# cvxopt/cvxopt

Hardware: NVIDIA H100
Metric: kkt_factor_solve_gflops_fp64 (higher is better)
Workload: dtype f64

## Files before the change

### cvxopt_b200/csrc/chol.cu

```cuda
#include "common.cuh"
#include <cstdlib>

namespace cvxb {

namespace {

constexpr int PB = 8;
constexpr int SP = 12;
constexpr int LDM = NB + 4;
constexpr int POTF2_SMEM = (NB * LDM + NB * SP + 4 * 80) * 8;
constexpr int kGroup = 4;

template <int PAT>
__device__ __forceinline__ void sym_update(double (&acc)[4][8][2], const double *Ma, const double *Mb) {
#pragma unroll 2
    for (int kk = 0; kk < NB / 4; ++kk) {
        double a[4], bfr[8];
#pragma unroll
        for (int cf = 0; cf < 4; ++cf) a[cf] = -Ma[cf * 8 + kk * 4 * LDM];
#pragma unroll
        for (int rf = 0; rf < 8; ++rf) bfr[rf] = Mb[rf * 8 + kk * 4 * LDM];
#pragma unroll
        for (int mf = 0; mf < 2; ++mf)
#pragma unroll
            for (int rf = 0; rf < 8; ++rf) {
                if (PAT == 1 && rf < 2 * mf) continue;
                if (PAT == 2 && rf < 4 + 2 * mf) continue;
                dmma16x8x4(acc[2 * mf][rf][0], acc[2 * mf][rf][1], acc[2 * mf + 1][rf][0], acc[2 * mf + 1][rf][1],
                           a[2 * mf], a[2 * mf + 1], bfr[rf]);
            }
    }
}

__global__ void __launch_bounds__(256, 1)
potf2_inv_kernel(double *A, long long lda, int jb, double *inv, double *invT, int *info, int joff,
                 long long sA, long long sInv, const double *Tprev, long long ldt,
                 const double *invprev, unsigned long long *trace) {
    extern __shared__ __align__(16) double sm[];
    if (trace && threadIdx.x == 0) {
        unsigned long long t; asm volatile("mov.u64 %0, %%globaltimer;" : "=l"(t)); trace[0] = t;
    }
#define CVXB_STAMP(SLOT)                                                                    \
    if (trace && threadIdx.x == 0) {                                                        \
        unsigned long long t_; asm volatile("mov.u64 %0, %%globaltimer;" : "=l"(t_));       \
        trace[8 * 2048 + (SLOT)] = t_;                                                      \
    }
    A += (long long)blockIdx.x * sA; inv += (long long)blockIdx.x * sInv;
    invT += (long long)blockIdx.x * sInv; info += blockIdx.x;
    double *M = sm;
    double *P = M + NB * LDM;
    double *Dw = P + NB * SP;
    const int tid = threadIdx.x, lane = tid & 31, warp = tid >> 5;
    const int role = (0x72640531 >> (warp * 4)) & 7;
    const int wr = role & 1, wc = role >> 1;
    const int g4 = lane >> 2, t4 = lane & 3;

    double acc[4][8][2];
    if (Tprev != nullptr) {
#pragma unroll
        for (int cf = 0; cf < 4; ++cf)
#pragma unroll
            for (int rf = 0; rf < 8; ++rf) acc[cf][rf][0] = acc[cf][rf][1] = 0.0;
        const int kkmax = (wc + 1) * 8;
        {
            const bool v16 = ((ldt & 1) == 0) && ((reinterpret_cast<uintptr_t>(Tprev) & 15) == 0);
            if (v16) {
                for (int q = tid; q < NB * NB / 2; q += 256) {
                    const int c = q >> 6, r = (q & 63) * 2;
                    const int nb = (r + 1 < jb) ? 16 : (r < jb ? 8 : 0);
                    cp_async16(M + r + c * LDM, nb ? Tprev + r + (long long)c * ldt : Tprev, nb);
                }
            } else {
                for (int q = tid; q < NB * NB; q += 256) {
                    const int c = q >> 7, r = q & 127;
                    cp_async8(M + r + c * LDM, (r < jb) ? Tprev + r + (long long)c * ldt : Tprev, (r < jb) ? 8 : 0);
                }
            }
            cp_async_commit();
        }
        const double *ip = invprev + (wc * 32 + g4) + t4 * NB;
        double a0[4];
#pragma unroll
        for (int cf = 0; cf < 4; ++cf) a0[cf] = ip[cf * 8];
        cp_async_wait<0>();
        __syncthreads();
        const double *tq = M + (wr * 64 + g4) + t4 * LDM;
#pragma unroll 2
        for (int kk = 0; kk < kkmax; ++kk) {
            double a[4], bfr[8];
#pragma unroll
            for (int cf = 0; cf < 4; ++cf) a[cf] = a0[cf];
            if (kk + 1 < kkmax) {
#pragma unroll
                for (int cf = 0; cf < 4; ++cf) a0[cf] = ip[cf * 8 + (kk + 1) * 4 * NB];
            }
#pragma unroll
            for (int rf = 0; rf < 8; ++rf) bfr[rf] = tq[rf * 8 + kk * 4 * LDM];
#pragma unroll
            for (int mf = 0; mf < 2; ++mf)
#pragma unroll
                for (int rf = 0; rf < 8; ++rf)
                    dmma16x8x4(acc[2 * mf][rf][0], acc[2 * mf][rf][1], acc[2 * mf + 1][rf][0],
                               acc[2 * mf + 1][rf][1], a[2 * mf], a[2 * mf + 1], bfr[rf]);
        }
        __syncthreads();
#pragma unroll
        for (int cf = 0; cf < 4; ++cf)
#pragma unroll
            for (int rf = 0; rf < 8; ++rf)
#pragma unroll
                for (int e = 0; e < 2; ++e)
                    M[(wr * 64 + rf * 8 + t4 * 2 + e) + (wc * 32 + cf * 8 + g4) * LDM] = acc[cf][rf][e];
    }
    CVXB_STAMP(0)
#pragma unroll
    for (int cf = 0; cf < 4; ++cf)
#pragma unroll
        for (int rf = 0; rf < 8; ++rf)
#pragma unroll
            for (int e = 0; e < 2; ++e) {
                const int r = wr * 64 + rf * 8 + t4 * 2 + e, c = wc * 32 + cf * 8 + g4;
                double v = (r == c) ? 1.0 : 0.0;
                if (r < jb && c < jb && r >= c) v = A[r + (long long)c * lda];
                acc[cf][rf][e] = v;
            }
    __syncthreads();
    CVXB_STAMP(4)
    if (Tprev != nullptr) {
        const int d = wc - 2 * wr;
        const double *Ma = M + (wc * 32 + g4) + t4 * LDM;
        const double *Mb = M + (wr * 64 + g4) + t4 * LDM;
        if (d < 0) sym_update<0>(acc, Ma, Mb);
        else if (d == 0) sym_update<1>(acc, Ma, Mb);
        else if (d == 1) sym_update<2>(acc, Ma, Mb);
        __syncthreads();
    }
    CVXB_STAMP(1)
#pragma unroll 1
    for (int t = 0; t < NB / PB; ++t) {
      {
        const int c0 = t * PB;
        if (wc == (t >> 2)) {
#define CVXB_PUBLISH(CF)                                                          \
    _Pragma("unroll") for (int rf = 0; rf < 8; ++rf)                              \
        _Pragma("unroll") for (int e = 0; e < 2; ++e)                             \
            P[(wr * 64 + rf * 8 + t4 * 2 + e) * SP + g4] = acc[CF][rf][e];
            switch (t & 3) {
                case 0: CVXB_PUBLISH(0) break;
                case 1: CVXB_PUBLISH(1) break;
                case 2: CVXB_PUBLISH(2) break;
                default: CVXB_PUBLISH(3) break;
            }
#undef CVXB_PUBLISH
        }
        __syncthreads();
        if (warp == 0 && lane == 0) {
            double a[PB][PB];
#pragma unroll
            for (int i = 0; i < PB; ++i)
#pragma unroll
                for (int k = 0; k <= i; ++k) a[i][k] = P[(c0 + i) * SP + k];
            bool bad = false;
#pragma unroll
            for (int j = 0; j < PB; ++j) {
                const double piv = a[j][j];
                if (!(piv > 0.0) && !bad) {
                    atomicCAS(info, 0, joff + c0 + j + 1);
                    bad = true;
                }
                const double rs = rsqrt(piv);
                a[j][j] = piv * rs;
                Dw[64 + j] = rs;
#pragma unroll
                for (int i = j + 1; i < PB; ++i) a[i][j] *= rs;
#pragma unroll
                for (int k = j + 1; k < PB; ++k)
#pragma unroll
                    for (int i = k; i < PB; ++i) a[i][k] -= a[i][j] * a[k][j];
            }
#pragma unroll
            for (int i = 0; i < PB; ++i)
#pragma unroll
                for (int k = 0; k < PB; ++k) Dw[i * 8 + k] = (k <= i) ? a[i][k] : 0.0;
        }
        if (warp < 4) asm volatile("bar.sync 1, 128;" ::: "memory");
        if (warp < 4) {
            const double *D = Dw;
            const int r = warp * 32 + lane;
            double x[PB];
            if (r >= c0 + PB) {
#pragma unroll
                for (int j = 0; j < PB; ++j) x[j] = P[r * SP + j];
#pragma unroll
                for (int j = 0; j < PB; ++j) {
                    double v = x[j];
#pragma unroll
                    for (int k = 0; k < j; ++k) v -= x[k] * D[j * 8 + k];
                    x[j] = v * D[64 + j];
                }
            } else if (r >= c0) {
#pragma unroll
                for (int j = 0; j < PB; ++j) x[j] = (j <= r - c0) ? D[(r - c0) * 8 + j] : 0.0;
            } else {
#pragma unroll
                for (int j = 0; j < PB; ++j) x[j] = 0.0;
            }
#pragma unroll
            for (int j = 0; j < PB; ++j) P[r * SP + j] = x[j];
        }
        __syncthreads();
        if (wr * 8 + 7 > t && wc * 4 + 3 > t) {
            double a[4][2], bfr[8][2];
#pragma unroll
            for (int kk = 0; kk < 2; ++kk) {
#pragma unroll
                for (int cf = 0; cf < 4; ++cf) a[cf][kk] = -P[(wc * 32 + cf * 8 + g4) * SP + kk * 4 + t4];
#pragma unroll
                for (int rf = 0; rf < 8; ++rf) bfr[rf][kk] = P[(wr * 64 + rf * 8 + g4) * SP + kk * 4 + t4];
            }
#pragma unroll
            for (int mf = 0; mf < 2; ++mf) {
                if (wc * 4 + 2 * mf + 1 <= t) continue;
#pragma unroll
                for (int rf = 0; rf < 8; ++rf) {
                    dmma16x8x4(acc[2 * mf][rf][0], acc[2 * mf][rf][1], acc[2 * mf + 1][rf][0], acc[2 * mf + 1][rf][1],
                               a[2 * mf][0], a[2 * mf + 1][0], bfr[rf][0]);
                    dmma16x8x4(acc[2 * mf][rf][0], acc[2 * mf][rf][1], acc[2 * mf + 1][rf][0], acc[2 * mf + 1][rf][1],
                               a[2 * mf][1], a[2 * mf + 1][1], bfr[rf][1]);
                }
            }
        }
        for (int e = tid; e < NB * PB; e += 256) {
            const int r = e & (NB - 1), j = e >> 7;
            const double v = P[r * SP + j];
            M[r + (c0 + j) * LDM] = v;
            if (r >= c0 + j && r < jb && c0 + j < jb) A[r + (long long)(c0 + j) * lda] = v;
        }
        __syncthreads();
      }
    }

    CVXB_STAMP(2)
    {
        const int blk = warp * 2 + (lane >> 4);
        const int j = lane & 15;
        const int o = blk * PB;
        double x[PB];
        if (j < PB) {
#pragma unroll
            for (int i = 0; i < PB; ++i) {
                double v = (i == j) ? 1.0 : 0.0;
#pragma unroll
                for (int k = 0; k < i; ++k)
                    if (k >= j) v -= M[(o + i) + (o + k) * LDM] * x[k];
                x[i] = (i >= j) ? v / M[(o + i) + (o + i) * LDM] : 0.0;
            }
        }
        __syncwarp();
        if (j < PB) {
#pragma unroll
            for (int i = 0; i < PB; ++i) M[(o + i) + (o + j) * LDM] = x[i];
        }
    }
    __syncthreads();
    for (int s = PB; s < NB; s <<= 1) {
        const int sb = s / PB;
        const int tp = sb * sb;
        const int ntiles = (NB / (2 * s)) * tp;
#pragma unroll 1
        for (int phase = 0; phase < 2; ++phase) {
            for (int base = warp * 4; base < ntiles; base += 32) {
                double c[4][2];
                int oo[4], ti[4], tj[4];
#pragma unroll
                for (int u = 0; u < 4; ++u) {
                    const int idx = min(base + u, ntiles - 1);
                    const int pr = idx / tp, loc = idx - pr * tp;
                    ti[u] = loc % sb; tj[u] = loc / sb; oo[u] = pr * 2 * s;
                    c[u][0] = c[u][1] = 0.0;
                }
                for (int kb = 0; kb < sb; ++kb) {
#pragma unroll
                    for (int u = 0; u < 4; ++u) {
                        const bool live = phase == 0 ? (kb >= tj[u]) : (kb <= ti[u]);
                        if (!live) continue;
                        const int o = oo[u];
#pragma unroll
                        for (int kk = 0; kk < 2; ++kk) {
                            const int k = kb * 8 + kk * 4 + t4;
                            double af, bf;
                            if (phase == 0) {
                                af = M[(o + s + ti[u] * 8 + g4) + (o + k) * LDM];
                                bf = M[(o + k) + (o + tj[u] * 8 + g4) * LDM];
                            } else {
                                af = M[(o + s + ti[u] * 8 + g4) + (o + s + k) * LDM];
                                bf = M[(o + k) + (o + s + tj[u] * 8 + g4) * LDM];
                            }
                            dmma(c[u][0], c[u][1], af, bf);
                        }
                    }
                }
#pragma unroll
                for (int u = 0; u < 4; ++u) {
                    if (base + u >= ntiles) continue;
                    const int o = oo[u];
                    if (phase == 0) {
                        M[(o + ti[u] * 8 + g4) + (o + s + tj[u] * 8 + t4 * 2) * LDM] = c[u][0];
                        M[(o + ti[u] * 8 + g4) + (o + s + tj[u] * 8 + t4 * 2 + 1) * LDM] = c[u][1];
                    } else {
                        M[(o + s + ti[u] * 8 + g4) + (o + tj[u] * 8 + t4 * 2) * LDM] = -c[u][0];
                        M[(o + s + ti[u] * 8 + g4) + (o + tj[u] * 8 + t4 * 2 + 1) * LDM] = -c[u][1];
                    }
                }
            }
            __syncthreads();
        }
    }
    CVXB_STAMP(3)
    for (int e = tid; e < NB * NB; e += 256) {
        int i = e & (NB - 1), k = e >> 7;
        inv[e] = (i >= k) ? M[i + k * LDM] : 0.0;
        invT[e] = (k >= i) ? M[k + i * LDM] : 0.0;
    }
    if (trace && threadIdx.x == 0) {
        unsigned long long t; asm volatile("mov.u64 %0, %%globaltimer;" : "=l"(t)); trace[1] = t;
    }
}

constexpr int TR_CH = 32;
constexpr int TR_R = 5;
constexpr int TRSV_SMEM = (TR_R * NB * TR_CH + 4 * NB + 32 * 129) * 8;

template <bool TRANS, bool VEC>
__global__ void __launch_bounds__(256, 1)
trsv_kernel(int n, const double *__restrict__ L, long long ldl, const double *__restrict__ inv,
            const double *__restrict__ invT, double *b, int *flags, int epoch, long long sL,
            long long sInv, long long sb) {
    extern __shared__ __align__(16) double sm[];
    {
        const long long pb = blockIdx.y;
        L += pb * sL; inv += pb * sInv; invT += pb * sInv; b += pb * sb;
        flags += pb * ((n + NB - 1) / NB);
    }
    double *ring = sm;
    double *xs = ring + TR_R * NB * TR_CH;
    double *part = xs + NB;
    double *tvec = part + 2 * NB;
    double *part2 = tvec + NB;
    const int nblk = (n + NB - 1) / NB;
    const int tid = threadIdx.x, lane = tid & 31, warp = tid >> 5;
    const int bi = TRANS ? (nblk - 1 - (int)blockIdx.x) : (int)blockIdx.x;
    const int i0 = bi * NB;
    const int ni = min(NB, n - i0);
    const int r = tid & (NB - 1), half = tid >> 7;

    double ireg[64];
    {
        const double *ip = (TRANS ? invT : inv) + (long long)bi * NB * NB + r + (long long)(half * 64) * NB;
#pragma unroll
        for (int k = 0; k < 64; ++k) ireg[k] = ip[k * NB];
    }

    const double bown = (tid < ni) ? b[i0 + tid] : 0.0;
    const int nb_dep = TRANS ? (nblk - 1 - bi) : bi;
    const int nchunks = nb_dep * (NB / TR_CH);
    auto issue = [&](int q) {
        const int jj = q / (NB / TR_CH), cc = q % (NB / TR_CH);
        const int j = TRANS ? (nblk - 1 - jj) : jj;
        double *dst = ring + (q % TR_R) * (NB * TR_CH);
        const double *src;
        int nrows, ncols;
        if (!TRANS) { src = L + i0 + (long long)(j * NB + cc * TR_CH) * ldl; nrows = ni; ncols = TR_CH; }
        else { src = L + (long long)j * NB + (long long)(i0 + cc * TR_CH) * ldl; nrows = min(NB, n - j * NB); ncols = min(TR_CH, ni - cc * TR_CH); }
        if (VEC) {
#pragma unroll
            for (int it = 0; it < 8; ++it) {
                const int e = tid + it * 256;
                const int c = e >> 6, rr = (e & 63) * 2;
                const int rem = nrows - rr;
                const int bytes = (c < ncols) ? (rem >= 2 ? 16 : (rem == 1 ? 8 : 0)) : 0;
                cp_async16(dst + c * NB + rr, bytes ? (src + rr + (long long)c * ldl) : L, bytes);
            }
        } else {
#pragma unroll
            for (int it = 0; it < 16; ++it) {
                const int e = tid + it * 256;
                const int c = e >> 7, rr = e & 127;
                const int bytes = (c < ncols && rr < nrows) ? 8 : 0;
                cp_async8(dst + c * NB + rr, bytes ? (src + rr + (long long)c * ldl) : L, bytes);
            }
        }
    };
#pragma unroll
    for (int q = 0; q < TR_R - 1; ++q) {
        if (q < nchunks) issue(q);
        cp_async_commit();
    }

    double acc = 0.0;
    double accc[16];
#pragma unroll
    for (int q = 0; q < 16; ++q) accc[q] = 0.0;

    for (int jj = 0; jj < nb_dep; ++jj) {
        const int j = TRANS ? (nblk - 1 - jj) : jj;
        if (tid == 0) while (ld_acquire(flags + j) != epoch) { }
        __syncthreads();
        if (tid < NB) xs[tid] = (j * NB + tid < n) ? __ldcg(b + j * NB + tid) : 0.0;
#pragma unroll
        for (int cc = 0; cc < NB / TR_CH; ++cc) {
            const int q = jj * (NB / TR_CH) + cc;
            cp_async_wait<TR_R - 2>();
            __syncthreads();
            {
                const int nq = q + TR_R - 1;
                if (nq < nchunks) issue(nq);
                cp_async_commit();
            }
            const double *ch = ring + (q % TR_R) * (NB * TR_CH);
            if (!TRANS) {
#pragma unroll
                for (int c = 0; c < 16; ++c)
                    acc += ch[(half * 16 + c) * NB + r] * xs[cc * TR_CH + half * 16 + c];
            } else {
#pragma unroll
                for (int qc = 0; qc < 4; ++qc) {
                    const double *col = ch + (warp * 4 + qc) * NB;
                    double a = 0.0;
#pragma unroll
                    for (int rr = 0; rr < 4; ++rr) a += col[lane + rr * 32] * xs[lane + rr * 32];
                    accc[cc * 4 + qc] += a;
                }
            }
        }
    }
    cp_async_wait<0>();
    __syncthreads();
    if (!TRANS) {
        part[half * NB + r] = acc;
        __syncthreads();
        if (tid < NB) tvec[tid] = (tid < ni) ? (bown - part[tid] - part[NB + tid]) : 0.0;
        __syncthreads();
    } else {
#pragma unroll
        for (int q = 0; q < 16; ++q) {
            const int c = (q >> 2) * TR_CH + warp * 4 + (q & 3);
            part2[lane * 129 + c] = accc[q];
        }
        __syncthreads();
        if (tid < NB) {
            double sacc = 0.0;
#pragma unroll 8
            for (int l = 0; l < 32; ++l) sacc += part2[l * 129 + tid];
            tvec[tid] = (tid < ni) ? (bown - sacc) : 0.0;
        }
        __syncthreads();
    }
    double a2 = 0.0;
#pragma unroll
    for (int k = 0; k < 64; ++k) a2 += ireg[k] * tvec[half * 64 + k];
    part[half * NB + r] = a2;
    __syncthreads();
    if (tid < ni) b[i0 + tid] = part[tid] + part[NB + tid];
    __threadfence();
    __syncthreads();
    if (tid == 0) st_release(flags + bi, epoch);
}

std::atomic<int> g_trsv_epoch{0};

__global__ void __launch_bounds__(256)
transpose_panel_kernel(const double *__restrict__ W, long long ldw, int rows, double *__restrict__ WT, long long ldt) {
    __shared__ double t[32][33];
    const int r0 = blockIdx.x * 32, k0 = blockIdx.y * 32, tx = threadIdx.x, ty = threadIdx.y;
#pragma unroll
    for (int i = ty; i < 32; i += 8)
        if (r0 + tx < rows) t[i][tx] = W[r0 + tx + (long long)(k0 + i) * ldw];
    __syncthreads();
#pragma unroll
    for (int i = ty; i < 32; i += 8)
        if (r0 + i < rows) WT[k0 + tx + (long long)(r0 + i) * ldt] = t[tx][i];
}

}

int chol_work_create(CholWork &w) {
    int least = 0, greatest = 0;
    CVXB_CUDA(cudaDeviceGetStreamPriorityRange(&least, &greatest));
    CVXB_CUDA(cudaStreamCreateWithPriority(&w.panel_stream, cudaStreamNonBlocking, greatest));
    CVXB_CUDA(cudaStreamCreateWithPriority(&w.trsm_stream, cudaStreamNonBlocking, greatest));
    CVXB_CUDA(cudaStreamCreateWithPriority(&w.update_stream, cudaStreamNonBlocking, least));
    CVXB_CUDA(cudaStreamCreateWithPriority(&w.near_stream, cudaStreamNonBlocking, greatest));
    CVXB_CUDA(cudaEventCreateWithFlags(&w.ev_end_t, cudaEventDisableTiming));
    CVXB_CUDA(cudaEventCreateWithFlags(&w.ev_end_n, cudaEventDisableTiming));
    CVXB_CUDA(cudaEventCreateWithFlags(&w.ev_start, cudaEventDisableTiming));
    CVXB_CUDA(cudaEventCreateWithFlags(&w.ev_end_p, cudaEventDisableTiming));
    CVXB_CUDA(cudaEventCreateWithFlags(&w.ev_end_u, cudaEventDisableTiming));
    CVXB_TRY(w.d_info.alloc(1));
    CVXB_CUDA(cudaMemset(w.d_info.p, 0, sizeof(int)));
    CVXB_TRY(w.d_flags.alloc(4096));
    CVXB_CUDA(cudaMemset(w.d_flags.p, 0, 4096 * sizeof(int)));
    CVXB_TRY(w.splitk_ws.alloc(dmma_gemm_splitk_ws_doubles()));
    CVXB_CUDA(cudaFuncSetAttribute(potf2_inv_kernel, cudaFuncAttributeMaxDynamicSharedMemorySize,
                                   POTF2_SMEM));
    CVXB_CUDA(cudaFuncSetAttribute(trsv_kernel<true, true>, cudaFuncAttributeMaxDynamicSharedMemorySize, TRSV_SMEM));
    CVXB_CUDA(cudaFuncSetAttribute(trsv_kernel<true, false>, cudaFuncAttributeMaxDynamicSharedMemorySize, TRSV_SMEM));
    CVXB_CUDA(cudaFuncSetAttribute(trsv_kernel<false, true>, cudaFuncAttributeMaxDynamicSharedMemorySize, TRSV_SMEM));
    CVXB_CUDA(cudaFuncSetAttribute(trsv_kernel<false, false>, cudaFuncAttributeMaxDynamicSharedMemorySize, TRSV_SMEM));
    return 0;
}

CholWork::~CholWork() {
    for (cudaStream_t s : {panel_stream, update_stream, trsm_stream, near_stream}) if (s) cudaStreamDestroy(s);
    for (auto &g : graphs) if (g.exec) cudaGraphExecDestroy(g.exec);
    for (cudaEvent_t e : {ev_end_t, ev_end_n, ev_start, ev_end_p, ev_end_u}) if (e) cudaEventDestroy(e);
    for (auto *v : {&ev_dg, &ev_tr, &ev_c0, &ev_na, &ev_nb, &ev_n})
        for (cudaEvent_t e : *v) cudaEventDestroy(e);
}

static int potrf_enqueue(int n, double *A, int lda, double *inv, CholWork &w, cudaStream_t st) {
    if (n <= 0) return 0;
    const int nblk = (n + NB - 1) / NB;
    if (w.panel_rows < n) {
        for (auto &g : w.graphs) if (g.exec) cudaGraphExecDestroy(g.exec);
        w.graphs.clear();
        for (DevBuf<double> &pb : w.panel) pb.reset();
        for (DevBuf<double> &gb : w.group) gb.reset();
        const int rows = (n + 1) & ~1;
        for (DevBuf<double> &pb : w.panel) CVXB_TRY(pb.alloc((size_t)rows * NB));
        for (DevBuf<double> &gb : w.group) CVXB_TRY(gb.alloc((size_t)rows * kGroup * NB));
        w.panel_rows = rows;
    }
    while ((int)w.ev_dg.size() < nblk) {
        cudaEvent_t e[6];
        for (int i = 0; i < 6; ++i) CVXB_CUDA(cudaEventCreateWithFlags(&e[i], cudaEventDisableTiming));
        w.ev_dg.push_back(e[0]); w.ev_tr.push_back(e[1]); w.ev_c0.push_back(e[2]);
        w.ev_na.push_back(e[3]); w.ev_nb.push_back(e[4]); w.ev_n.push_back(e[5]);
    }
    if (getenv("CVXB_TRACE") && !w.trace.p) CVXB_TRY(w.trace.alloc(8 * 4096));
    unsigned long long *trace = w.trace.p;
    if (trace) CVXB_CUDA(cudaMemsetAsync(trace, 0, 8 * 4096 * sizeof(unsigned long long), st));
    const int ldw = w.panel_rows;
    const int ldg = kGroup * NB;
    cudaStream_t D = w.panel_stream, T = w.trsm_stream, U = w.update_stream, N = w.near_stream;
    CVXB_CUDA(cudaMemsetAsync(w.d_info.p, 0, sizeof(int), st));
    CVXB_CUDA(cudaEventRecord(w.ev_start, st));
    for (cudaStream_t s : {D, T, U, N}) CVXB_CUDA(cudaStreamWaitEvent(s, w.ev_start, 0));
    auto update = [&](int lo, int hi, const double *X, int ldx, bool kmajor, int K, unsigned long long *tr,
                      cudaStream_t s) -> int {
        double *Acc = A + (long long)lo * NB * (1 + (long long)lda);
        GemmDesc u;
        u.M = n - lo * NB; u.N = (hi * NB < n ? hi * NB : n) - lo * NB; u.K = K;
        u.X = X; u.ldx = ldx; u.x_kmajor = kmajor;
        u.Y = X; u.ldy = ldx; u.y_kmajor = kmajor;
        u.D = Acc; u.ldd = lda; u.C = Acc; u.ldc = lda;
        u.alpha = -1.0; u.beta = 1.0; u.lower_only = true;
        u.trace = tr;
        return dmma_gemm(u, s);
    };
    auto wait_col = [&](cudaStream_t s, int c) -> int {
        const int p = c - 2, g0 = kGroup * (c / kGroup);
        if (p < 0) return 0;
        if (p >= g0) CVXB_CUDA(cudaStreamWaitEvent(s, w.ev_na[p], 0));
        if (g0 > 0) CVXB_CUDA(cudaStreamWaitEvent(s, w.ev_nb[p < g0 - 1 ? p : g0 - 1], 0));
        return 0;
    };
    for (int jb = 0; jb < nblk; ++jb) {
        const int j = jb * NB;
        const int wj = (n - j < NB) ? (n - j) : NB;
        const int m = n - j - wj;
        double *Ajj = A + j + (long long)j * lda;
        double *invj = inv + (long long)jb * NB * NB;
        double *invTj = inv + (long long)(nblk + jb) * NB * NB;
        double *Wp = w.panel[jb & 1].p;
        if (jb >= 2) CVXB_CUDA(cudaStreamWaitEvent(D, w.ev_c0[jb - 2], 0));
        CVXB_TRY(wait_col(D, jb));
        const double *Tprev = jb > 0 ? A + j + (long long)(j - NB) * lda : nullptr;
        const double *invprev = jb > 0 ? inv + (long long)(jb - 1) * NB * NB : nullptr;
        potf2_inv_kernel<<<1, 256, POTF2_SMEM, D>>>(Ajj, lda, wj, invj, invTj, w.d_info.p, j, 0, 0, Tprev,
                                                     lda, invprev, trace ? trace + 8 * jb : nullptr);
        count_launch();
        CVXB_LAUNCH_CHECK();
        CVXB_CUDA(cudaEventRecord(w.ev_dg[jb], D));
        auto copy_back_prev = [&]() -> int {
            if (jb == 0) return 0;
            const int jp = j - NB, mp = n - j;
            CVXB_CUDA(cudaMemcpy2DAsync(A + j + (long long)jp * lda, (size_t)lda * sizeof(double),
                                        w.panel[(jb - 1) & 1].p, (size_t)ldw * sizeof(double),
                                        (size_t)mp * sizeof(double), NB, cudaMemcpyDeviceToDevice, T));
            return 0;
        };
        if (m <= 0) {
            CVXB_CUDA(cudaStreamWaitEvent(T, w.ev_dg[jb], 0));
            CVXB_TRY(copy_back_prev());
            break;
        }
        double *A21 = Ajj + wj;
        double *A22 = A21 + (long long)wj * lda;
        CVXB_CUDA(cudaStreamWaitEvent(T, w.ev_dg[jb], 0));
        if (jb >= 2) CVXB_CUDA(cudaStreamWaitEvent(T, w.ev_n[jb - 2], 0));
        {
            GemmDesc g;
            g.M = m; g.N = wj; g.K = wj;
            g.X = A21; g.ldx = lda; g.x_kmajor = false;
            g.Y = invj; g.ldy = NB; g.y_kmajor = false;
            g.C = Wp; g.ldc = ldw;
            g.trace = trace ? trace + 8 * jb + 2 : nullptr;
            CVXB_TRY(dmma_gemm(g, T));
        }
        CVXB_CUDA(cudaEventRecord(w.ev_tr[jb], T));
        CVXB_TRY(wait_col(T, jb + 1));
        const int wn = (m < NB) ? m : NB;
        if (m > wn) {
            GemmDesc c;
            c.M = m - wn; c.N = wn; c.K = wj;
            c.X = Wp + wn; c.Y = Wp;
            c.ldx = ldw; c.x_kmajor = false;
            c.ldy = ldw; c.y_kmajor = false;
            c.D = A22 + wn; c.ldd = lda; c.C = A22 + wn; c.ldc = lda;
            c.alpha = -1.0; c.beta = 1.0;
            c.trace = trace ? trace + 8 * jb + 4 : nullptr;
            CVXB_TRY(dmma_gemm(c, T));
        }
        CVXB_CUDA(cudaEventRecord(w.ev_c0[jb], T));
        CVXB_TRY(copy_back_prev());
        const int q = jb / kGroup, s = jb % kGroup, gq = kGroup * (q + 1);
        double *Wg = w.group[q & 1].p;
        unsigned long long *tr_near = trace ? trace + 8 * jb + 6 : nullptr;
        CVXB_CUDA(cudaStreamWaitEvent(N, w.ev_tr[jb], 0));
        if (s == 0 && jb > 0) CVXB_CUDA(cudaStreamWaitEvent(N, w.ev_nb[jb - 1], 0));
        {
            const int lo = jb + 2, hi = gq < nblk ? gq : nblk;
            if (lo < hi) CVXB_TRY(update(lo, hi, Wp + (lo - jb - 1) * NB, ldw, false, NB, tr_near, N));
        }
        CVXB_CUDA(cudaEventRecord(w.ev_na[jb], N));
        if (gq < nblk) {
            const int rows = n - gq * NB;
            transpose_panel_kernel<<<dim3((rows + 31) / 32, NB / 32), dim3(32, 8), 0, N>>>(
                Wp + (gq - jb - 1) * NB, ldw, rows, Wg + s * NB, ldg);
            count_launch();
            CVXB_LAUNCH_CHECK();
        }
        CVXB_CUDA(cudaEventRecord(w.ev_n[jb], N));
        if (gq < nblk) {
            CVXB_CUDA(cudaStreamWaitEvent(U, w.ev_n[jb], 0));
            const int lo = gq > jb + 2 ? gq : jb + 2, hi = gq + kGroup < nblk ? gq + kGroup : nblk;
            if (lo < hi) CVXB_TRY(update(lo, hi, Wg + s * NB + (long long)(lo - gq) * NB * ldg, ldg, true, NB, tr_near, U));
            CVXB_CUDA(cudaEventRecord(w.ev_nb[jb], U));
            if (s == kGroup - 1 && gq + kGroup < nblk)
                CVXB_TRY(update(gq + kGroup, nblk, Wg + (long long)kGroup * NB * ldg, ldg, true, kGroup * NB,
                                trace ? trace + 8 * 2048 + 8 * jb + 5 : nullptr, U));
        }
    }
    CVXB_CUDA(cudaEventRecord(w.ev_end_p, D));
    CVXB_CUDA(cudaEventRecord(w.ev_end_u, U));
    CVXB_CUDA(cudaEventRecord(w.ev_end_t, T));
    CVXB_CUDA(cudaEventRecord(w.ev_end_n, N));
    for (cudaEvent_t e : {w.ev_end_p, w.ev_end_u, w.ev_end_t, w.ev_end_n}) CVXB_CUDA(cudaStreamWaitEvent(st, e, 0));
    return 0;
}

int potrf_lower(int n, double *A, int lda, double *inv, CholWork &w, cudaStream_t st) {
    if (n <= 0) return 0;
    if (w.graph_failed || n > 4096) return potrf_enqueue(n, A, lda, inv, w, st);
    CholWork::GraphEntry *ent = nullptr;
    for (auto &g : w.graphs)
        if (g.n == n && g.A == A && g.lda == lda && g.inv == inv) { ent = &g; break; }
    if (ent && ent->exec) {
        CVXB_CUDA(cudaGraphLaunch(ent->exec, st));
        count_launch(ent->launches);
        return 0;
    }
    if (!ent) {
        if (w.graphs.size() >= 4) {
            for (auto &g : w.graphs) if (g.exec) cudaGraphExecDestroy(g.exec);
            w.graphs.clear();
        }
        CholWork::GraphEntry g;
        g.n = n; g.A = A; g.lda = lda; g.inv = inv;
        w.graphs.push_back(g);
        return potrf_enqueue(n, A, lda, inv, w, st);
    }
    const unsigned long long l0 = g_launches.load();
    if (cudaStreamBeginCapture(st, cudaStreamCaptureModeRelaxed) != cudaSuccess) {
        cudaGetLastError();
        w.graph_failed = true;
        return potrf_enqueue(n, A, lda, inv, w, st);
    }
    const int rc = potrf_enqueue(n, A, lda, inv, w, st);
    cudaGraph_t graph = nullptr;
    const cudaError_t ce = cudaStreamEndCapture(st, &graph);
    const int captured = (int)(g_launches.load() - l0);
    g_launches.fetch_sub((unsigned long long)captured);
    if (rc != 0 || ce != cudaSuccess || !graph) {
        cudaGetLastError();
        if (graph) cudaGraphDestroy(graph);
        w.graph_failed = true;
        return potrf_enqueue(n, A, lda, inv, w, st);
    }
    cudaGraphExec_t exec = nullptr;
    if (cudaGraphInstantiate(&exec, graph, 0) != cudaSuccess || !exec) {
        cudaGetLastError();
        cudaGraphDestroy(graph);
        w.graph_failed = true;
        return potrf_enqueue(n, A, lda, inv, w, st);
    }
    cudaGraphDestroy(graph);
    ent->exec = exec;
    ent->launches = captured;
    CVXB_CUDA(cudaGraphLaunch(exec, st));
    count_launch(captured);
    return 0;
}

int trsv_lower(int n, const double *L, int ldl, const double *inv, double *b, bool trans,
               CholWork &w, cudaStream_t st, int batch, long long sL, long long sInv, long long sb) {
    if (n <= 0 || batch <= 0) return 0;
    const int nblk = (n + NB - 1) / NB;
    const size_t nflags = (size_t)nblk * batch;
    if (nflags > w.d_flags.n) {
        w.d_flags.reset();
        CVXB_TRY(w.d_flags.alloc(nflags));
        CVXB_CUDA(cudaMemsetAsync(w.d_flags.p, 0, nflags * sizeof(int), st));
    }
    const int epoch = g_trsv_epoch.fetch_add(1) + 1;
    const double *invT = inv + (long long)nblk * NB * NB;
    const bool vec = ((uintptr_t)L % 16 == 0) && (ldl % 2 == 0) && (batch == 1 || sL % 2 == 0);
    dim3 grid(nblk, batch);
#define TRSV_LAUNCH(T, V) trsv_kernel<T, V><<<grid, 256, TRSV_SMEM, st>>>(n, L, ldl, inv, invT, b, w.d_flags.p, epoch, sL, sInv, sb)
    if (trans) { if (vec) TRSV_LAUNCH(true, true); else TRSV_LAUNCH(true, false); }
    else       { if (vec) TRSV_LAUNCH(false, true); else TRSV_LAUNCH(false, false); }
#undef TRSV_LAUNCH
    count_launch();
    CVXB_LAUNCH_CHECK();
    return 0;
}

int potrs_lower(int n, const double *L, int ldl, const double *inv, double *b, CholWork &w,
                cudaStream_t st, int batch, long long sL, long long sInv, long long sb) {
    CVXB_TRY(trsv_lower(n, L, ldl, inv, b, false, w, st, batch, sL, sInv, sb));
    CVXB_TRY(trsv_lower(n, L, ldl, inv, b, true, w, st, batch, sL, sInv, sb));
    return 0;
}

namespace {
__global__ void copy2d_batched_kernel(const double *src, long long lds, long long ssrc, double *dst,
                                      long long ldd, long long sdst, int rows, int cols) {
    const long long pb = blockIdx.z;
    const int r = blockIdx.x * blockDim.x + threadIdx.x, c = blockIdx.y;
    if (r < rows && c < cols) dst[pb * sdst + r + (long long)c * ldd] = src[pb * ssrc + r + (long long)c * lds];
}
}

int potrf_lower_batched(int n, double *A, int lda, long long sA, double *inv, long long sInv,
                        int batch, int *d_info, double *panel, int ldw, cudaStream_t st) {
    if (n <= 0 || batch <= 0) return 0;
    const int nblk = (n + NB - 1) / NB;
    CVXB_CUDA(cudaMemsetAsync(d_info, 0, (size_t)batch * sizeof(int), st));
    const long long sW = (long long)ldw * NB;
    for (int jb = 0; jb < nblk; ++jb) {
        const int j = jb * NB;
        const int wj = (n - j < NB) ? (n - j) : NB;
        const int m = n - j - wj;
        double *Ajj = A + j + (long long)j * lda;
        double *invj = inv + (long long)jb * NB * NB;
        double *invTj = inv + (long long)(nblk + jb) * NB * NB;
        potf2_inv_kernel<<<batch, 256, POTF2_SMEM, st>>>(Ajj, lda, wj, invj, invTj, d_info, j, sA, sInv, nullptr, 0,
                                                        nullptr, nullptr);
        count_launch();
        CVXB_LAUNCH_CHECK();
        if (m <= 0) break;
        double *A21 = Ajj + wj;
        double *A22 = A21 + (long long)wj * lda;
        GemmDesc g;
        g.M = m; g.N = wj; g.K = wj;
        g.X = A21; g.ldx = lda; g.x_kmajor = false; g.sX = sA;
        g.Y = invj; g.ldy = NB; g.y_kmajor = false; g.sY = sInv;
        g.C = panel; g.ldc = ldw; g.sC = sW; g.batch = batch;
        CVXB_TRY(dmma_gemm(g, st));
        GemmDesc u;
        u.M = m; u.N = m; u.K = wj;
        u.X = panel; u.ldx = ldw; u.x_kmajor = false; u.sX = sW;
        u.Y = panel; u.ldy = ldw; u.y_kmajor = false; u.sY = sW;
        u.D = A22; u.ldd = lda; u.sD = sA; u.C = A22; u.ldc = lda; u.sC = sA;
        u.alpha = -1.0; u.beta = 1.0; u.lower_only = true; u.batch = batch;
        CVXB_TRY(dmma_gemm(u, st));
        dim3 cg((m + 255) / 256, wj, batch);
        copy2d_batched_kernel<<<cg, 256, 0, st>>>(panel, ldw, sW, A21, lda, sA, m, wj);
        count_launch();
        CVXB_LAUNCH_CHECK();
    }
    return 0;
}

}
```

Measured before the change: 40410.

## Pipeline panel factorization with producer warps and double-buffered rank-8 updates

Restructures the diagonal-block Cholesky plus inverse kernel. Two dedicated warps now factor each 8-column panel and do its triangular solve. The remaining warps apply the rank-8 trailing updates from a double-buffered panel and publish the next panel early through named barriers, so factorization overlaps with the update. The previous inverse block is staged into shared memory with cp.async, and the triangular inverse doubling levels are unrolled per level with 16x8 DMMA tiles. Zero-filling of inv/invT moves earlier, so the final write skips the zero halves. This adds complex barrier-count logic and uses more shared memory, which risks deadlock or correctness bugs.

```diff
diff --git a/cvxopt_b200/csrc/chol.cu b/cvxopt_b200/csrc/chol.cu
--- a/cvxopt_b200/csrc/chol.cu
+++ b/cvxopt_b200/csrc/chol.cu
@@ -8,7 +8,11 @@
 constexpr int PB = 8;
 constexpr int SP = 12;
 constexpr int LDM = NB + 4;
-constexpr int POTF2_SMEM = (NB * LDM + NB * SP + 4 * 80) * 8;
+constexpr int LDI = 36;
+constexpr int IPS_DOUBLES = LDI * 32 * (1 + 2 + 3 + 4);
+constexpr int POTF2_SMEM = (NB * LDM + IPS_DOUBLES) * 8;
+static_assert(3 * NB * SP <= IPS_DOUBLES, "panel buffers alias the staged inverse");
+static_assert(POTF2_SMEM <= 227 * 1024, "potf2_inv_kernel exceeds the opt-in shared memory of one CTA");
 constexpr int kGroup = 4;
 
 template <int PAT>
@@ -29,6 +33,79 @@
                 dmma16x8x4(acc[2 * mf][rf][0], acc[2 * mf][rf][1], acc[2 * mf + 1][rf][0], acc[2 * mf + 1][rf][1],
                            a[2 * mf], a[2 * mf + 1], bfr[rf]);
             }
+    }
+}
+
+template <int PAT>
+__device__ __forceinline__ void rank8_update(double (&acc)[4][8][2], const double *Q, int wr, int wc, int g4, int t4,
+                                             int t, int mfmask) {
+    double a[4][2], bfr[8][2];
+#pragma unroll
+    for (int kk = 0; kk < 2; ++kk) {
+#pragma unroll
+        for (int cf = 0; cf < 4; ++cf) a[cf][kk] = -Q[(wc * 32 + cf * 8 + g4) * SP + kk * 4 + t4];
+#pragma unroll
+        for (int rf = 0; rf < 8; ++rf) bfr[rf][kk] = Q[(wr * 64 + rf * 8 + g4) * SP + kk * 4 + t4];
+    }
+#pragma unroll
+    for (int mf = 0; mf < 2; ++mf) {
+        if (!(mfmask >> mf & 1) || wc * 4 + 2 * mf + 1 <= t) continue;
+#pragma unroll
+        for (int rf = 0; rf < 8; ++rf) {
+            if (PAT == 1 && rf < 2 * mf) continue;
+            if (PAT == 2 && rf < 4 + 2 * mf) continue;
+#pragma unroll
+            for (int kk = 0; kk < 2; ++kk)
+                dmma16x8x4(acc[2 * mf][rf][0], acc[2 * mf][rf][1], acc[2 * mf + 1][rf][0], acc[2 * mf + 1][rf][1],
+                           a[2 * mf][kk], a[2 * mf + 1][kk], bfr[rf][kk]);
+        }
+    }
+}
+
+template <int S>
+__device__ __forceinline__ void inverse_level(double *M, int warp, int g4, int t4) {
+    constexpr int SB = S / 8, PER = S / 16, TPP = SB * SB / 2;
+#pragma unroll
+    for (int phase = 0; phase < 2; ++phase) {
+        double c[PER][4];
+        int o[PER], ti[PER], tj[PER];
+#pragma unroll
+        for (int u = 0; u < PER; ++u) {
+            const int idx = warp * PER + u, pr = idx / TPP, loc = idx % TPP;
+            ti[u] = (loc % (SB / 2)) * 2; tj[u] = loc / (SB / 2); o[u] = pr * 2 * S;
+            c[u][0] = c[u][1] = c[u][2] = c[u][3] = 0.0;
+        }
+        const int ko = phase ? S : 0;
+#pragma unroll
+        for (int kb = 0; kb < SB; ++kb) {
+#pragma unroll
+            for (int u = 0; u < PER; ++u) {
+                const bool live = phase == 0 ? (kb >= tj[u]) : (kb <= ti[u] + 1);
+                if (!live) continue;
+#pragma unroll
+                for (int kk = 0; kk < 2; ++kk) {
+                    const int k = kb * 8 + kk * 4 + t4;
+                    const double *ar = M + (o[u] + S + ti[u] * 8 + g4) + (o[u] + ko + k) * LDM;
+                    double a0 = ar[0];
+                    const double a1 = ar[8];
+                    if (phase == 1 && kb > ti[u]) a0 = 0.0;
+                    const double b = M[(o[u] + k) + (o[u] + ko + tj[u] * 8 + g4) * LDM];
+                    dmma16x8x4(c[u][0], c[u][1], c[u][2], c[u][3], a0, a1, b);
+                }
+            }
+        }
+#pragma unroll
+        for (int u = 0; u < PER; ++u)
+#pragma unroll
+            for (int h = 0; h < 2; ++h)
+#pragma unroll
+                for (int e = 0; e < 2; ++e) {
+                    if (phase == 0)
+                        M[(o[u] + ti[u] * 8 + h * 8 + g4) + (o[u] + S + tj[u] * 8 + t4 * 2 + e) * LDM] = c[u][2 * h + e];
+                    else
+                        M[(o[u] + S + ti[u] * 8 + h * 8 + g4) + (o[u] + tj[u] * 8 + t4 * 2 + e) * LDM] = -c[u][2 * h + e];
+                }
+        __syncthreads();
     }
 }
 
@@ -48,12 +125,14 @@
     A += (long long)blockIdx.x * sA; inv += (long long)blockIdx.x * sInv;
     invT += (long long)blockIdx.x * sInv; info += blockIdx.x;
     double *M = sm;
-    double *P = M + NB * LDM;
-    double *Dw = P + NB * SP;
+    double *IPS = M + NB * LDM;
+    double *P = IPS;
+    double *Qb = IPS + NB * SP;
     const int tid = threadIdx.x, lane = tid & 31, warp = tid >> 5;
     const int role = (0x72640531 >> (warp * 4)) & 7;
     const int wr = role & 1, wc = role >> 1;
     const int g4 = lane >> 2, t4 = lane & 3;
+    const int d = wc - 2 * wr;
 
     double acc[4][8][2];
     if (Tprev != nullptr) {
@@ -76,24 +155,31 @@
                     cp_async8(M + r + c * LDM, (r < jb) ? Tprev + r + (long long)c * ldt : Tprev, (r < jb) ? 8 : 0);
                 }
             }
+            const bool i16 = (reinterpret_cast<uintptr_t>(invprev) & 15) == 0;
+            for (int q = tid; q < IPS_DOUBLES / LDI * 16; q += 256) {
+                const int col = q >> 4, rr = (q & 15) * 2;
+                const int b = col < 32 ? 0 : (col < 96 ? 1 : (col < 192 ? 2 : 3));
+                const int k = col - 16 * b * (b + 1);
+                double *dst = IPS + LDI * (16 * b * (b + 1) + k) + rr;
+                const double *src = invprev + (b * 32 + rr) + (long long)k * NB;
+                if (i16) {
+                    cp_async16(dst, src, 16);
+                } else {
+                    cp_async8(dst, src, 8);
+                    cp_async8(dst + 1, src + 1, 8);
+                }
+            }
             cp_async_commit();
         }
-        const double *ip = invprev + (wc * 32 + g4) + t4 * NB;
-        double a0[4];
-#pragma unroll
-        for (int cf = 0; cf < 4; ++cf) a0[cf] = ip[cf * 8];
         cp_async_wait<0>();
         __syncthreads();
+        const double *ip = IPS + LDI * (16 * wc * (wc + 1)) + g4 + t4 * LDI;
         const double *tq = M + (wr * 64 + g4) + t4 * LDM;
 #pragma unroll 2
         for (int kk = 0; kk < kkmax; ++kk) {
             double a[4], bfr[8];
 #pragma unroll
-            for (int cf = 0; cf < 4; ++cf) a[cf] = a0[cf];
-            if (kk + 1 < kkmax) {
-#pragma unroll
-                for (int cf = 0; cf < 4; ++cf) a0[cf] = ip[cf * 8 + (kk + 1) * 4 * NB];
-            }
+            for (int cf = 0; cf < 4; ++cf) a[cf] = ip[cf * 8 + kk * 4 * LDI];
 #pragma unroll
             for (int rf = 0; rf < 8; ++rf) bfr[rf] = tq[rf * 8 + kk * 4 * LDM];
 #pragma unroll
@@ -124,121 +210,109 @@
                 if (r < jb && c < jb && r >= c) v = A[r + (long long)c * lda];
                 acc[cf][rf][e] = v;
             }
+    for (int e = tid; e < NB * NB; e += 256) {
+        const int i = e & (NB - 1), k = e >> 7;
+        if (i < k) inv[e] = 0.0;
+        if (k < i) invT[e] = 0.0;
+    }
     __syncthreads();
     CVXB_STAMP(4)
     if (Tprev != nullptr) {
-        const int d = wc - 2 * wr;
         const double *Ma = M + (wc * 32 + g4) + t4 * LDM;
         const double *Mb = M + (wr * 64 + g4) + t4 * LDM;
         if (d < 0) sym_update<0>(acc, Ma, Mb);
         else if (d == 0) sym_update<1>(acc, Ma, Mb);
         else if (d == 1) sym_update<2>(acc, Ma, Mb);
-        __syncthreads();
-    }
-    CVXB_STAMP(1)
-#pragma unroll 1
-    for (int t = 0; t < NB / PB; ++t) {
-      {
-        const int c0 = t * PB;
-        if (wc == (t >> 2)) {
+    }
 #define CVXB_PUBLISH(CF)                                                          \
     _Pragma("unroll") for (int rf = 0; rf < 8; ++rf)                              \
         _Pragma("unroll") for (int e = 0; e < 2; ++e)                             \
             P[(wr * 64 + rf * 8 + t4 * 2 + e) * SP + g4] = acc[CF][rf][e];
-            switch (t & 3) {
-                case 0: CVXB_PUBLISH(0) break;
-                case 1: CVXB_PUBLISH(1) break;
-                case 2: CVXB_PUBLISH(2) break;
-                default: CVXB_PUBLISH(3) break;
-            }
-#undef CVXB_PUBLISH
-        }
-        __syncthreads();
-        if (warp == 0 && lane == 0) {
-            double a[PB][PB];
+    if (wc == 0) { CVXB_PUBLISH(0) }
+    __syncthreads();
+    CVXB_STAMP(1)
+    if (warp == 4 || warp == 5) {
+        const int lt = tid - 128;
+#pragma unroll 1
+        for (int t = 0; t < NB / PB; ++t) {
+            const int c0 = t * PB;
+            if (t > 0) {
+                const int cnt = 64 + (t < 8 ? 64 : 32);
+                asm volatile("bar.sync 1, %0;" ::"r"(cnt) : "memory");
+            }
+            double *Q = Qb + (t & 1) * NB * SP;
+            double a[PB][PB], x[2][PB];
 #pragma unroll
             for (int i = 0; i < PB; ++i)
 #pragma unroll
                 for (int k = 0; k <= i; ++k) a[i][k] = P[(c0 + i) * SP + k];
-            bool bad = false;
+#pragma unroll
+            for (int h = 0; h < 2; ++h)
+#pragma unroll
+                for (int j = 0; j < PB; ++j) x[h][j] = P[(lt + 64 * h) * SP + j];
 #pragma unroll
             for (int j = 0; j < PB; ++j) {
                 const double piv = a[j][j];
-                if (!(piv > 0.0) && !bad) {
-                    atomicCAS(info, 0, joff + c0 + j + 1);
-                    bad = true;
-                }
+                if (lt == 0 && !(piv > 0.0)) atomicCAS(info, 0, joff + c0 + j + 1);
                 const double rs = rsqrt(piv);
                 a[j][j] = piv * rs;
-                Dw[64 + j] = rs;
 #pragma unroll
                 for (int i = j + 1; i < PB; ++i) a[i][j] *= rs;
 #pragma unroll
-                for (int k = j + 1; k < PB; ++k)
+                for (int h = 0; h < 2; ++h) x[h][j] *= rs;
+#pragma unroll
+                for (int k = j + 1; k < PB; ++k) {
+#pragma unroll
+                    for (int h = 0; h < 2; ++h) x[h][k] -= x[h][j] * a[k][j];
 #pragma unroll
                     for (int i = k; i < PB; ++i) a[i][k] -= a[i][j] * a[k][j];
-            }
-#pragma unroll
-            for (int i = 0; i < PB; ++i)
-#pragma unroll
-                for (int k = 0; k < PB; ++k) Dw[i * 8 + k] = (k <= i) ? a[i][k] : 0.0;
-        }
-        if (warp < 4) asm volatile("bar.sync 1, 128;" ::: "memory");
-        if (warp < 4) {
-            const double *D = Dw;
-            const int r = warp * 32 + lane;
-            double x[PB];
-            if (r >= c0 + PB) {
-#pragma unroll
-                for (int j = 0; j < PB; ++j) x[j] = P[r * SP + j];
+                }
+            }
+#pragma unroll
+            for (int h = 0; h < 2; ++h) {
+                const int r = lt + 64 * h;
 #pragma unroll
                 for (int j = 0; j < PB; ++j) {
-                    double v = x[j];
-#pragma unroll
-                    for (int k = 0; k < j; ++k) v -= x[k] * D[j * 8 + k];
-                    x[j] = v * D[64 + j];
-                }
-            } else if (r >= c0) {
-#pragma unroll
-                for (int j = 0; j < PB; ++j) x[j] = (j <= r - c0) ? D[(r - c0) * 8 + j] : 0.0;
-            } else {
-#pragma unroll
-                for (int j = 0; j < PB; ++j) x[j] = 0.0;
-            }
-#pragma unroll
-            for (int j = 0; j < PB; ++j) P[r * SP + j] = x[j];
-        }
-        __syncthreads();
-        if (wr * 8 + 7 > t && wc * 4 + 3 > t) {
-            double a[4][2], bfr[8][2];
-#pragma unroll
-            for (int kk = 0; kk < 2; ++kk) {
-#pragma unroll
-                for (int cf = 0; cf < 4; ++cf) a[cf][kk] = -P[(wc * 32 + cf * 8 + g4) * SP + kk * 4 + t4];
-#pragma unroll
-                for (int rf = 0; rf < 8; ++rf) bfr[rf][kk] = P[(wr * 64 + rf * 8 + g4) * SP + kk * 4 + t4];
-            }
-#pragma unroll
-            for (int mf = 0; mf < 2; ++mf) {
-                if (wc * 4 + 2 * mf + 1 <= t) continue;
-#pragma unroll
-                for (int rf = 0; rf < 8; ++rf) {
-                    dmma16x8x4(acc[2 * mf][rf][0], acc[2 * mf][rf][1], acc[2 * mf + 1][rf][0], acc[2 * mf + 1][rf][1],
-                               a[2 * mf][0], a[2 * mf + 1][0], bfr[rf][0]);
-                    dmma16x8x4(acc[2 * mf][rf][0], acc[2 * mf][rf][1], acc[2 * mf + 1][rf][0], acc[2 * mf + 1][rf][1],
-                               a[2 * mf][1], a[2 * mf + 1][1], bfr[rf][1]);
-                }
-            }
-        }
-        for (int e = tid; e < NB * PB; e += 256) {
-            const int r = e & (NB - 1), j = e >> 7;
-            const double v = P[r * SP + j];
-            M[r + (c0 + j) * LDM] = v;
-            if (r >= c0 + j && r < jb && c0 + j < jb) A[r + (long long)(c0 + j) * lda] = v;
-        }
-        __syncthreads();
-      }
-    }
+                    const double v = (r >= c0 + j) ? x[h][j] : 0.0;
+                    Q[r * SP + j] = v;
+                    M[r + (c0 + j) * LDM] = v;
+                    if (r >= c0 + j && r < jb && c0 + j < jb) A[r + (long long)(c0 + j) * lda] = v;
+                }
+            }
+            asm volatile("bar.sync 2, 256;" ::: "memory");
+        }
+    } else {
+        asm volatile("bar.sync 2, 256;" ::: "memory");
+#pragma unroll 1
+        for (int t = 0; t < NB / PB - 1; ++t) {
+            const double *Q = Qb + (t & 1) * NB * SP;
+            const int tn = t + 1;
+            const bool pub = wc == (tn >> 2) && (tn < 8 || wr == 1);
+            const int first = pub ? 1 << ((tn & 3) >> 1) : 3;
+            if (wr * 8 + 7 > t && wc * 4 + 3 > t) {
+                if (d < 0) rank8_update<0>(acc, Q, wr, wc, g4, t4, t, first);
+                else if (d == 0) rank8_update<1>(acc, Q, wr, wc, g4, t4, t, first);
+                else rank8_update<2>(acc, Q, wr, wc, g4, t4, t, first);
+            }
+            if (pub) {
+                switch (tn & 3) {
+                    case 0: CVXB_PUBLISH(0) break;
+                    case 1: CVXB_PUBLISH(1) break;
+                    case 2: CVXB_PUBLISH(2) break;
+                    default: CVXB_PUBLISH(3) break;
+                }
+                const int cnt = 64 + (tn < 8 ? 64 : 32);
+                asm volatile("bar.arrive 1, %0;" ::"r"(cnt) : "memory");
+                if (wr * 8 + 7 > t && wc * 4 + 3 > t) {
+                    if (d < 0) rank8_update<0>(acc, Q, wr, wc, g4, t4, t, 3 ^ first);
+                    else if (d == 0) rank8_update<1>(acc, Q, wr, wc, g4, t4, t, 3 ^ first);
+                    else rank8_update<2>(acc, Q, wr, wc, g4, t4, t, 3 ^ first);
+                }
+            }
+            asm volatile("bar.sync 2, 256;" ::: "memory");
+        }
+    }
+#undef CVXB_PUBLISH
 
     CVXB_STAMP(2)
     {
@@ -262,65 +336,36 @@
             for (int i = 0; i < PB; ++i) M[(o + i) + (o + j) * LDM] = x[i];
         }
     }
+    __syncwarp();
+    {
+        const int o = warp * 2 * PB;
+        double c0 = 0.0, c1 = 0.0;
+#pragma unroll
+        for (int kk = 0; kk < 2; ++kk) {
+            const int k = kk * 4 + t4;
+            dmma(c0, c1, M[(o + PB + g4) + (o + k) * LDM], M[(o + k) + (o + g4) * LDM]);
+        }
+        M[(o + g4) + (o + PB + t4 * 2) * LDM] = c0;
+        M[(o + g4) + (o + PB + t4 * 2 + 1) * LDM] = c1;
+        __syncwarp();
+        c0 = c1 = 0.0;
+#pragma unroll
+        for (int kk = 0; kk < 2; ++kk) {
+            const int k = kk * 4 + t4;
+            dmma(c0, c1, M[(o + PB + g4) + (o + PB + k) * LDM], M[(o + k) + (o + PB + g4) * LDM]);
+        }
+        M[(o + PB + g4) + (o + t4 * 2) * LDM] = -c0;
+        M[(o + PB + g4) + (o + t4 * 2 + 1) * LDM] = -c1;
+    }
     __syncthreads();
-    for (int s = PB; s < NB; s <<= 1) {
-        const int sb = s / PB;
-        const int tp = sb * sb;
-        const int ntiles = (NB / (2 * s)) * tp;
-#pragma unroll 1
-        for (int phase = 0; phase < 2; ++phase) {
-            for (int base = warp * 4; base < ntiles; base += 32) {
-                double c[4][2];
-                int oo[4], ti[4], tj[4];
-#pragma unroll
-                for (int u = 0; u < 4; ++u) {
-                    const int idx = min(base + u, ntiles - 1);
-                    const int pr = idx / tp, loc = idx - pr * tp;
-                    ti[u] = loc % sb; tj[u] = loc / sb; oo[u] = pr * 2 * s;
-                    c[u][0] = c[u][1] = 0.0;
-                }
-                for (int kb = 0; kb < sb; ++kb) {
-#pragma unroll
-                    for (int u = 0; u < 4; ++u) {
-                        const bool live = phase == 0 ? (kb >= tj[u]) : (kb <= ti[u]);
-                        if (!live) continue;
-                        const int o = oo[u];
-#pragma unroll
-                        for (int kk = 0; kk < 2; ++kk) {
-                            const int k = kb * 8 + kk * 4 + t4;
-                            double af, bf;
-                            if (phase == 0) {
-                                af = M[(o + s + ti[u] * 8 + g4) + (o + k) * LDM];
-                                bf = M[(o + k) + (o + tj[u] * 8 + g4) * LDM];
-                            } else {
-                                af = M[(o + s + ti[u] * 8 + g4) + (o + s + k) * LDM];
-                                bf = M[(o + k) + (o + s + tj[u] * 8 + g4) * LDM];
-                            }
-                            dmma(c[u][0], c[u][1], af, bf);
-                        }
-                    }
-                }
-#pragma unroll
-                for (int u = 0; u < 4; ++u) {
-                    if (base + u >= ntiles) continue;
-                    const int o = oo[u];
-                    if (phase == 0) {
-                        M[(o + ti[u] * 8 + g4) + (o + s + tj[u] * 8 + t4 * 2) * LDM] = c[u][0];
-                        M[(o + ti[u] * 8 + g4) + (o + s + tj[u] * 8 + t4 * 2 + 1) * LDM] = c[u][1];
-                    } else {
-                        M[(o + s + ti[u] * 8 + g4) + (o + tj[u] * 8 + t4 * 2) * LDM] = -c[u][0];
-                        M[(o + s + ti[u] * 8 + g4) + (o + tj[u] * 8 + t4 * 2 + 1) * LDM] = -c[u][1];
-                    }
-                }
-            }
-            __syncthreads();
-        }
-    }
+    inverse_level<16>(M, warp, g4, t4);
+    inverse_level<32>(M, warp, g4, t4);
+    inverse_level<64>(M, warp, g4, t4);
     CVXB_STAMP(3)
     for (int e = tid; e < NB * NB; e += 256) {
         int i = e & (NB - 1), k = e >> 7;
-        inv[e] = (i >= k) ? M[i + k * LDM] : 0.0;
-        invT[e] = (k >= i) ? M[k + i * LDM] : 0.0;
+        if (i >= k) inv[e] = M[i + k * LDM];
+        if (k >= i) invT[e] = M[k + i * LDM];
     }
     if (trace && threadIdx.x == 0) {
         unsigned long long t; asm volatile("mov.u64 %0, %%globaltimer;" : "=l"(t)); trace[1] = t;
```

Measured after the change: 41080, median of 6. 1.7% higher.
